# DredderGun/accbpg_and_fw

Hardware: AMD Instinct MI355X
Metric: D-opt iters/sec (m=2048,n=32768) (higher is better)
Workload: dtype f64; 1 GPU; D_opt_design(2048,32768) abpg_gain gamma=2 fp64, one independent instance per GPU; instances=1, instances_per_gpu=1, seeds=1..1, window=transient: iterations 5..161 from x0 = 1/n, linear_gram=False

## Files before the change

accbpg_and_fw_amd/_lib.py:

```python
from __future__ import annotations

import ctypes as C
import os

_HERE = os.path.dirname(os.path.abspath(__file__))
LIB_PATH = os.environ.get("ACCBPG_HIP_LIB") or os.path.join(_HERE, "lib", "libaccbpg_hip.so")

OK, ERR_ASSERT, ERR_NOT_PD, ERR_HIP, ERR_ARG = 0, 1, 2, 3, 4

_lib = None


class FwProbe(C.Structure):
    _fields_ = [("i", C.c_int64), ("j", C.c_int64), ("w_i", C.c_double), ("w_j", C.c_double),
                ("x_j", C.c_double), ("logdet_H", C.c_double), ("q_prev", C.c_double)]


class FwStep(C.Structure):
    _fields_ = [("i", C.c_int64), ("j", C.c_int64), ("w_i", C.c_double), ("w_j", C.c_double), ("x_j", C.c_double),
                ("q_prev", C.c_double), ("p", C.c_int64), ("xscale", C.c_double), ("xadd", C.c_double),
                ("hcoef", C.c_double), ("hdiv", C.c_double), ("kind", C.c_int32), ("status", C.c_int32)]


FW_RUN_MAX = 1024
# ... 94 lines not shown
    "accbpg_symnmf_func_grad": (C.c_int, [_P, _P, C.c_int, C.POINTER(C.c_double), _P]),
    "accbpg_symnmf_plan": (C.c_int, [_P, C.POINTER(C.c_int64)]),
    "accbpg_quartic_prox_stage": (C.c_int, [_P, _P, C.c_double, C.c_double, C.c_int, C.c_double, C.c_int64, _P,
                                            C.POINTER(C.c_double), _P, _P]),
    "accbpg_quartic_ls_terms": (C.c_int, [_P, _P, _P, _P, _P, C.c_int64, C.POINTER(C.c_double), _P, _P]),
    "accbpg_lmo_l2_ball": (C.c_int, [_P, C.c_int, _P, C.c_double, C.c_double, C.c_double, C.c_int64, _P,
                                     C.POINTER(C.c_double), _P, _P]),
    "accbpg_lmo_linf_ball": (C.c_int, [_P, C.c_int, _P, C.c_double, C.c_double, C.c_int64, _P, _P]),
    "accbpg_burg_reg_div_prox": (C.c_int, [C.c_int, _P, _P, C.c_double, C.c_double, C.c_int64, _P, _P]),
    "accbpg_vec_dot": (C.c_int, [_P, _P, C.c_int64, C.POINTER(C.c_double), _P, _P]),
    "accbpg_combine_ls_terms": (C.c_int, [C.c_int, C.c_double, _P, C.c_double, _P, C.c_double, _P, _P, C.c_int64, _P,
                                          C.POINTER(C.c_double), _P, _P]),
    "accbpg_burg_simplex_prox_acc": (C.c_int, [_P, C.c_double, _P, C.c_double, C.c_double, C.c_int64, _P, _P, _P,
                                               C.POINTER(C.c_int), _P]),
    "accbpg_lmo_l2_ball_pos": (C.c_int, [_P, _P, C.c_double, C.c_double, C.c_int64, _P, C.POINTER(C.c_double), _P, _P]),
    "accbpg_dopt_profile_enable": (C.c_int, [_P, C.c_int]),
    "accbpg_dopt_profile_read": (C.c_int, [_P, C.c_int, C.POINTER(C.c_double), C.POINTER(C.c_int64)]),
    "accbpg_dopt_profile_reset": (C.c_int, [_P]),
    "accbpg_debug_pipe_probe": (C.c_int, [C.c_int, C.c_int, C.POINTER(C.c_double), _P]),
    "accbpg_mfma_f64_peak": (C.c_int, [C.c_int, C.POINTER(C.c_double), _P]),
    "accbpg_dopt_factor_in_small_launches": (C.c_int, [_P, C.c_int]),
    "accbpg_debug_chol_variant": (C.c_int, [_P, C.c_int]),
    "accbpg_debug_plan_flags": (C.c_int, [C.c_int]),
    "accbpg_debug_chol_trace": (C.c_int, [_P, _P, C.c_int, C.POINTER(C.c_int64)]),
    "accbpg_debug_gram_variant": (C.c_int, [_P, _P, C.c_int, C.c_int, C.POINTER(C.c_double)]),
    "accbpg_debug_grad_variant": (C.c_int, [_P, _P, C.c_int, C.c_int, C.POINTER(C.c_double)]),
    "accbpg_test_gemm": (C.c_int, [_P, C.c_int64, _P, C.c_int64, _P, C.c_int64, C.c_int64, C.c_int64,
                                   C.c_int64, C.c_int, C.c_double, C.c_double, C.c_int, _P]),
}

EXPORTS = tuple(sorted(_SIGS))


def load():
    global _lib
    if _lib is not None:
        return _lib
    if not os.path.exists(LIB_PATH):
        raise ImportError(
            "accbpg_and_fw_amd: %s is missing -- build it with "
            "`make -C accbpg_and_fw_amd/csrc` or `python -c 'import __graft_entry__ as g; g.build()'`. "
            "There is no CPU fallback." % LIB_PATH)
    lib = C.CDLL(LIB_PATH)
    for name, (res, args) in _SIGS.items():
        fn = getattr(lib, name)
        fn.restype = res
# ... 21 lines not shown
```

accbpg_and_fw_amd/csrc/capi.hip:

```cpp
#include <stdarg.h>
#include <string.h>
#include <stdlib.h>
#include <algorithm>

#include "internal.h"
#include "reduce.hpp"

namespace accbpg {

static thread_local char g_err[512] = "";

void set_last_error(const char* fmt, ...) {
    va_list ap;
    va_start(ap, fmt);
    vsnprintf(g_err, sizeof(g_err), fmt, ap);
    va_end(ap);
}

void note_tiles_fallback(const char* where) {
    static bool said = false;
    if (said) return;
    said = true;
    fprintf(stderr, "libaccbpg_hip: %s: the one-launch Cholesky abandoned a wait (another process on this GPU, or fewer "
                    "workgroups resident than the occupancy query promised); this handle factors with one launch per block "
// ... 461 lines not shown
}

extern "C" int accbpg_test_gemm(const double* A_dev, int64_t lda, const double* B_dev, int64_t ldb, double* C_dev,
                                int64_t ldc, int64_t M, int64_t N, int64_t K, int b_kmajor, double alpha,
                                double beta, int config, void* stream) {
    if (!A_dev || !B_dev || !C_dev || M <= 0 || N <= 0 || K <= 0) return ACCBPG_ERR_ARG;
    return launch_test_gemm(A_dev, lda, B_dev, ldb, C_dev, ldc, M, N, K, b_kmajor, alpha, beta, config,
                            (hipStream_t)stream);
}

extern "C" int accbpg_dopt_factor_in_small_launches(accbpg_dopt* h, int on) {
    if (!h || on < 0 || on > 2) return ACCBPG_ERR_ARG;
    const int64_t T = (h->m + NB - 1) / NB;
    value_forget(h);
    h->chol_tiles_off = on == 1 || (on == 2 && T * (T + 1) / 2 >= h->num_cu);
    return ACCBPG_OK;
}

extern "C" int accbpg_debug_plan_flags(int flags) {
    set_plan_flags(flags);
    return ACCBPG_OK;
}

extern "C" int accbpg_debug_chol_variant(accbpg_dopt* h, int bits) {
    if (!h) return ACCBPG_ERR_ARG;
    value_forget(h);
    h->chol_dbg = bits & 63;
    h->chol_tiles_off = (bits & 64) != 0;
    if (bits & 2048) h->chol_tiles_off = true;
    h->chol_stall_test = (bits & 128) ? 1 : 0;
    h->chol_spin_limit = (bits & 128) ? 200000 : 20000000;
    h->kern_variant = (bits >> 30) & 3;
    if (bits & 256) h->use_glds = false;
    if (bits & 512) h->use_glds = true;
    if (bits & 2048) {
        h->chol_two_level_T = (bits >> 12) & 0xfff;
        if ((bits >> 24) & 0x3f) h->chol_nk = (bits >> 24) & 0x3f;
    }
    return ACCBPG_OK;
}

extern "C" int accbpg_debug_chol_trace(accbpg_dopt* h, const double* gram_dev, int with_inverse, int64_t* stamps_host) {
    if (!h || !gram_dev || !stamps_host) return ACCBPG_ERR_ARG;
    if (!chol_tiles_usable(h)) {
        set_last_error("accbpg_debug_chol_trace: the one-launch Cholesky is not in use for this handle");
        return ACCBPG_ERR_ARG;
// ... 28 lines not shown
```

accbpg_and_fw_amd/csrc/dopt_kernels.hip:

```cpp
#include <mutex>
#include <unordered_map>
#include <type_traits>

#include "internal.h"
#include "mfma_tile.hpp"

namespace accbpg {

struct GramSeg {
    int64_t row0, col0, kb, ke;
    bool dual, whole;
};
constexpr int GRAM_RMAX = 4;
template <class T>
__device__ __forceinline__ GramSeg gram_segment(const TileRC* __restrict__ tiles, int64_t kiters, int64_t it,
                                                int64_t it1) {
    const int e = (int)(it / kiters);
    const int64_t off = it - (int64_t)e * kiters;
    const TileRC tr = tiles[e];
    GramSeg g;
    if (tr.d1 < 0) {
        g.row0 = (int64_t)tr.rb * T::BM; g.col0 = (int64_t)tr.cb * T::BN;
        g.kb = off; g.ke = min(kiters, off + (it1 - it));
        g.dual = false;
// ... 757 lines not shown
template <class T, int CV = 0>
__device__ __forceinline__ void colnorm_glds_body(
    const double* __restrict__ W, int64_t ldw, const double* __restrict__ V, int64_t ldv, int64_t m, int64_t n,
    double* __restrict__ out, double sign) {
    if constexpr (CV == COLNORM_CV) colnorm_phases_body<T>(W, ldw, V, ldv, m, n, out, sign);
    else colnorm_restart_body<T, CV>(W, ldw, V, ldv, m, n, out, sign);
}

template <class T, int CV = 0>
__global__ __launch_bounds__(NTHREADS, 1) void colnorm_glds_kernel(
    const double* __restrict__ W, int64_t ldw, const double* __restrict__ V, int64_t ldv, int64_t m, int64_t n,
    double* __restrict__ out, double sign) {
    colnorm_glds_body<T, CV>(W, ldw, V, ldv, m, n, out, sign);
}
template <class T>
__global__ __launch_bounds__(NTHREADS, 1) void colnorm_glds_batch_kernel(
    const BatchInst* __restrict__ bt, BatchAct act, int64_t ldw, int64_t ldv, int64_t m, int64_t n,
    double* __restrict__ outbase, int64_t ldo, double sign) {
    const int inst = act.idx[blockIdx.y];
    const BatchInst bi = bt[inst];
    colnorm_glds_body<T, COLNORM_CV>(bi.Wbuf, ldw, bi.V, ldv, m, n, outbase + (int64_t)inst * ldo, sign);
}

template <class T>
__device__ __forceinline__ void gemm_ops_body(const GemmOp op) {
    extern __shared__ __attribute__((aligned(16))) double lds[];
    const int64_t row0 = (int64_t)blockIdx.y * T::BM, col0 = (int64_t)blockIdx.x * T::BN;
    if (row0 >= op.M || col0 >= op.N) return;
    if (op.lower_only && col0 > row0 + T::BM - 1) return;
    const bool va = ((reinterpret_cast<uintptr_t>(op.A) & 15) == 0) && ((op.lda & 1) == 0);
    const bool vb = ((reinterpret_cast<uintptr_t>(op.B) & 15) == 0) && ((op.ldb & 1) == 0);
    T t;
    t.zero();
    int64_t ksteps = (op.K + BK - 1) / BK;
    int64_t ks0 = 0;
    if (op.tri & 1) ks0 = max((int64_t)0, col0 - op.koff) / BK;
    if (op.tri & 2) ksteps = min(ksteps, max((int64_t)0, row0 + T::BM - op.koff + BK - 1) / BK);
    if (ks0 >= ksteps) {
        t.store_C(op.C, op.ldc, row0, col0, op.M, op.N, op.alpha, op.beta, op.lower_only != 0);
        return;
    }
    auto gload = [&](int64_t ks) {
        t.gload_A(op.A, op.lda, row0, op.M, ks * BK, op.K, va);
        if constexpr (T::BKM) t.gload_B_km(op.B, op.ldb, col0, op.N, ks * BK, op.K, vb);
        else t.gload_B_kc(op.B, op.ldb, col0, op.N, ks * BK, op.K, vb);
    };
    gload(ks0);
    t.sstore(lds);
    __syncthreads();
    int cur = 0;
    for (int64_t ks = ks0; ks < ksteps; ++ks) {
        const bool more = ks + 1 < ksteps;
        if (more) gload(ks + 1);
        t.compute(lds + cur * T::STAGE_ELEMS);
        if (more) t.sstore(lds + (cur ^ 1) * T::STAGE_ELEMS);
        __syncthreads();
        cur ^= 1;
    }
    t.store_C(op.C, op.ldc, row0, col0, op.M, op.N, op.alpha, op.beta, op.lower_only != 0);
}

template <class T>
__global__ __launch_bounds__(NTHREADS, 2) void gemm_ops_kernel(const GemmOp* __restrict__ ops) {
    gemm_ops_body<T>(ops[blockIdx.z]);
}
template <class T>
__global__ __launch_bounds__(NTHREADS, 2) void gemm_ops_batch_kernel(const GemmOp* __restrict__ ops, int per_inst, int begin,
                                                                    int count, BatchAct act) {
    const int a = blockIdx.z / count, o = blockIdx.z - a * count;
    gemm_ops_body<T>(ops[(int64_t)act.idx[a] * per_inst + begin + o]);
}

__device__ __forceinline__ void gemm_reduce_body(const RedOp r) {
    const int64_t total = (int64_t)r.M * r.N;
    const int64_t stride = (int64_t)gridDim.x * 256 * 2;
    for (int64_t e = 2 * ((int64_t)blockIdx.x * 256 + threadIdx.x); e < total; e += stride) {
        double2 acc = *reinterpret_cast<const double2*>(r.P + e);
        for (int p = 1; p < r.ns; ++p) {
            const double2 v = *reinterpret_cast<const double2*>(r.P + (int64_t)p * total + e);
            acc.x += v.x;
            acc.y += v.y;
        }
        const int64_t row = e / r.N, col = e - row * r.N;
        *reinterpret_cast<double2*>(r.C + row * r.ldc + col) = acc;
    }
}
__global__ __launch_bounds__(256) void gemm_reduce_kernel(const RedOp* __restrict__ reds) { gemm_reduce_body(reds[blockIdx.y]); }
__global__ __launch_bounds__(256) void gemm_reduce_batch_kernel(const RedOp* __restrict__ reds, int per_inst, int begin, int count,
                                                               BatchAct act) {
    const int a = blockIdx.y / count, o = blockIdx.y - a * count;
    gemm_reduce_body(reds[(int64_t)act.idx[a] * per_inst + begin + o]);
}

// ... 1119 lines not shown

void prof_begin(accbpg_dopt* h, ProfKind k) {
    if (!h->prof_on) return;
    ProfSlot& p = h->prof[k];
    if (p.used + 2 > p.ev.size()) {
        hipEvent_t a, b;
        hipEventCreate(&a);
        hipEventCreate(&b);
        p.ev.push_back(a);
        p.ev.push_back(b);
    }
    hipEventRecord(p.ev[p.used], h->stream);
}
void prof_end(accbpg_dopt* h, ProfKind k) {
    if (!h->prof_on) return;
    ProfSlot& p = h->prof[k];
    hipEventRecord(p.ev[p.used + 1], h->stream);
    p.used += 2;
    p.launches += 1;
}

static int g_plan_flags = 0;
void set_plan_flags(int flags) { g_plan_flags = flags; }

int build_plans(accbpg_dopt* h) {
    const int64_t m = h->m;
    const bool interior256 = h->vec_ok && (m % 256 == 0) && (h->n % BK == 0);
    const int BM = h->big ? TileBig<false>::BM : TileSmall<false>::BM;
    const int BN = h->big ? TileBig<false>::BN : TileSmall<false>::BN;
    std::vector<TileRC> tl;
    const int nrb = (int)((m + BM - 1) / BM), ncb = (int)((m + BN - 1) / BN);
    h->gram_chunks = 1;
    h->gram_nc = h->n;
    constexpr int64_t GRAM_NC = 32768;
    if (!(g_plan_flags & 4) && h->big && interior256 && h->use_glds && h->n >= 2 * GRAM_NC && h->n % GRAM_NC == 0) {
        h->gram_chunks = (int)(h->n / GRAM_NC);
        h->gram_nc = GRAM_NC;
        if (!(g_plan_flags & 8) && h->ldv * (int64_t)sizeof(double) >= (1 << 20)) {
            const size_t bytes = sizeof(double) * (size_t)m * (size_t)h->n;
            if (hipMalloc(&h->Vblk, bytes) == hipSuccess) {
                for (int c = 0; c < h->gram_chunks; ++c)
                    ACC_HIP(hipMemcpy2DAsync(h->Vblk + (size_t)c * m * GRAM_NC, sizeof(double) * GRAM_NC,
                                             h->V + (size_t)c * GRAM_NC, sizeof(double) * (size_t)h->ldv,
                                             sizeof(double) * GRAM_NC, (size_t)m, hipMemcpyDeviceToDevice, h->stream));
                ACC_HIP(hipStreamSynchronize(h->stream));
            } else {
// ... 257 lines not shown
        h->chol_tiles_grid = (int)jobs.size();
        h->chol_slots = std::min(per_cu, 2) * h->num_cu;
        h->chol_tiles_ok = per_cu >= 1 && (int64_t)jobs.size() <= (int64_t)h->chol_slots;
        if (h->chol_tiles_ok) {
            ACC_HIP(hipMalloc(&h->chol_jobs, sizeof(CholJob) * jobs.size()));
            ACC_HIP(hipMemcpy(h->chol_jobs, jobs.data(), sizeof(CholJob) * jobs.size(), hipMemcpyHostToDevice));
            ACC_HIP(hipMalloc(&h->chol_ready, sizeof(int) * (size_t)(T * T + 5 * T)));
            ACC_HIP(hipMemset(h->chol_ready, 0, sizeof(int) * (size_t)(T * T + 5 * T)));
            ACC_HIP(hipMalloc(&h->chol_hand, sizeof(double) * (size_t)T * NB * NB));
            ACC_HIP(hipMalloc(&h->chol_aux, sizeof(double) * (size_t)T * CT_AUX));
            ACC_HIP(hipMalloc(&h->Gbuf, sizeof(double) * (size_t)m * m));
            ACC_HIP(hipMemset(h->Gbuf, 0, sizeof(double) * (size_t)m * m));
        }
    }

    ACC_TRY(set_lds(gram_streamk_kernel<TileBig<false, true>>, TileBig<false>::LDS_BYTES));
    ACC_TRY(set_lds(gram_streamk_kernel<TileBig<false, false>>, TileBig<false>::LDS_BYTES));
    ACC_TRY(set_lds(gram_streamk_kernel<TileSmall<false, true>>, TileSmall<false>::LDS_BYTES));
    ACC_TRY(set_lds(gram_streamk_kernel<TileSmall<false, false>>, TileSmall<false>::LDS_BYTES));
    ACC_TRY(set_lds(colnorm_kernel<TileBig<true, true>>, TileBig<true>::LDS_BYTES));
    ACC_TRY(set_lds(colnorm_kernel<TileBig<true, false>>, TileBig<true>::LDS_BYTES));
    ACC_TRY(set_lds(colnorm_kernel<TileSmall<true, true>>, TileSmall<true>::LDS_BYTES));
    ACC_TRY(set_lds(colnorm_kernel<TileSmall<true, false>>, TileSmall<true>::LDS_BYTES));
    ACC_TRY(set_lds(gemm_ops_kernel<TileSmall<true>>, TileSmall<true>::LDS_BYTES));
    ACC_TRY(set_lds(gemm_ops_kernel<TileSmall<false>>, TileSmall<false>::LDS_BYTES));
    ACC_TRY(set_lds(chol_step_kernel, CHOL_LDS_BYTES));
    ACC_TRY(set_lds(chol_syrk_kernel, SYRK_LDS_BYTES));
    ACC_TRY(set_lds(gemm_big_kernel<TileBig<true>>, TileBig<true>::LDS_BYTES));
    ACC_TRY(set_lds(gemm_big_kernel<TileBig<false>>, TileBig<false>::LDS_BYTES));
    return ACCBPG_OK;
}

template <class T>
static int gram_launch_t(accbpg_dopt* h, const double* x, double* gram) {
    if constexpr (!T::EDGE && T::BM == 256) {
        if (h->use_glds || h->has_duals) {
            const int64_t nc = h->gram_chunks > 1 ? h->gram_nc : h->n;
            for (int c = 0; c < h->gram_chunks; ++c) {
                const double* Vc = h->Vblk ? h->Vblk + (int64_t)c * h->m * nc : h->V + (int64_t)c * nc;
                const int64_t ldc = h->Vblk ? nc : h->ldv;
                const double* xc = x + (int64_t)c * nc;
                const double beta = c == 0 ? 0.0 : 1.0;
                const int all_slabs = h->gram_chunks > 1 ? 1 : 0;
                prof_begin(h, PROF_GRAM);
#define ACC_GRAM_ARGS Vc, ldc, h->m, nc, xc, h->tiles, h->wg_ranges, h->kiters, h->gram_nslot, h->slabs, gram, h->m, all_slabs
                if (h->kern_variant == 1)
                    ACC_LAUNCH_LDS((gram_streamk_glds_kernel<T, GRAM_GV ^ 128>), h->gram_grid, NTHREADS, T::G_LDS_BYTES, h->stream, ACC_GRAM_ARGS);
                else if (h->kern_variant == 3)
// ... 104 lines not shown
        if (interior) ACC_TRY((gram_launch_t<TileSmall<false, false>>(h, x, gram)));
        else ACC_TRY((gram_launch_t<TileSmall<false, true>>(h, x, gram)));
    }
    ACC_HIP(hipGetLastError());
    return ACCBPG_OK;
}

__global__ __launch_bounds__(256) void copy_kernel(double* __restrict__ dst, const double* __restrict__ src, size_t n) {
    const size_t stride = (size_t)gridDim.x * 256;
    for (size_t i = (size_t)blockIdx.x * 256 + threadIdx.x; i < n; i += stride) dst[i] = src[i];
}
int device_copy(double* dst, const double* src, size_t ndoubles, hipStream_t s) {
    if (ndoubles == 0 || dst == src) return ACCBPG_OK;
    size_t nb = (ndoubles + 255) / 256;
    if (nb > 4096) nb = 4096;
    copy_kernel<<<(unsigned)nb, 256, 0, s>>>(dst, src, ndoubles);
    ACC_HIP(hipGetLastError());
    return ACCBPG_OK;
}

int launch_gemm_ops(const GemmOp* ops_dev, int nops, int maxM, int maxN, bool b_kmajor, hipStream_t s) {
    if (nops <= 0 || maxM <= 0 || maxN <= 0) return ACCBPG_OK;
    dim3 grid((maxN + 63) / 64, (maxM + 63) / 64, nops);
    if (b_kmajor)
        gemm_ops_kernel<TileSmall<true>><<<grid, NTHREADS, TileSmall<true>::LDS_BYTES, s>>>(ops_dev);
    else
        gemm_ops_kernel<TileSmall<false>><<<grid, NTHREADS, TileSmall<false>::LDS_BYTES, s>>>(ops_dev);
    ACC_HIP(hipGetLastError());
    return ACCBPG_OK;
}

static std::mutex g_tiles_mu;
constexpr int TILES_RING = 16;
struct TilesRing {
    hipEvent_t ev[TILES_RING] = {};
    hipStream_t stream[TILES_RING] = {};
    int grid[TILES_RING] = {};
    long long issued = 0;
};
static TilesRing g_tiles[64];

bool chol_tiles_usable(const accbpg_dopt* h) {
    return h->chol_tiles_ok && !h->chol_tiles_off && (h->chol_dbg & 63) == 0;
}

static int launch_chol_tiles(accbpg_dopt* h, const double* src, double* A, double* Winv) {
    const int64_t m = h->m;
    const int T = (int)((m + NB - 1) / NB);
    CholInst ci;
    ci.src = src; ci.L = A; ci.Ldiag = h->Tbuf; ci.Winv = Winv; ci.logdet = h->dscal; ci.flags = h->dflag;
    ci.ready = h->chol_ready; ci.aux = h->chol_aux; ci.hand = h->chol_hand; ci.trace = h->chol_trace;
    const int dev = (h->device >= 0 && h->device < 64) ? h->device : 0;
// ... 161 lines not shown
        CholInst{}, b->chol_table[with_inverse ? 1 : 0], reinterpret_cast<const CholJob*>(h0->chol_jobs), m, m, T,
        h0->chol_spin_limit, 0, act);
    prof_end(h0, PROF_CHOL);
    ACC_HIP(hipGetLastError());
    {
        const int slot = (int)(ring.issued % TILES_RING);
        if (!ring.ev[slot]) ACC_HIP(hipEventCreateWithFlags(&ring.ev[slot], hipEventDisableTiming));
        ACC_HIP(hipEventRecord(ring.ev[slot], b->stream));
        ring.stream[slot] = b->stream;
        ring.grid[slot] = grid_all;
        ++ring.issued;
    }
    return ACCBPG_OK;
}

int launch_trtri_batch(accbpg_dopt_batch* b, const BatchAct& act) {
    accbpg_dopt* h0 = b->inst[0];
    prof_begin(h0, PROF_TRTRI);
    for (const accbpg_dopt::MergeStage& st : h0->merge_stages) {
        const int count = st.end - st.begin;
        if (count <= 0) continue;
        if (st.kind == 0) {
            dim3 grid((st.maxn + 63) / 64, (st.maxm + 63) / 64, count * act.n);
            gemm_ops_batch_kernel<TileSmall<true>><<<grid, NTHREADS, TileSmall<true>::LDS_BYTES, b->stream>>>(
                b->ops_all, b->ops_per_inst, st.begin, count, act);
        } else {
            int gx = (int)std::min<int64_t>(1024, ((int64_t)st.maxm / 2 + 255) / 256);
            gemm_reduce_batch_kernel<<<dim3(gx, count * act.n), 256, 0, b->stream>>>(b->red_all, b->red_per_inst, st.begin, count, act);
        }
    }
    prof_end(h0, PROF_TRTRI);
    ACC_HIP(hipGetLastError());
    return ACCBPG_OK;
}

int debug_grad_variant(accbpg_dopt* h, double* out, int var, int iters, double* ms_out) {
    using T = TileBig<true, false>;
    const bool vw = ((reinterpret_cast<uintptr_t>(h->Wbuf) & 15) == 0) && ((h->m & 1) == 0);
    if (!h->big || !h->use_glds || !vw || !h->vec_ok || h->m % 256 != 0 || h->n % 128 != 0) return ACCBPG_ERR_ARG;
    const int grid = (int)(h->n / T::BN), lds = T::G_LDS_BYTES + 4 * T::BN * 8;
    if (var != 0 && var != 3 && (var < 10 || var > 13)) return ACCBPG_ERR_ARG;
    hipEvent_t a, b;
    ACC_HIP(hipEventCreate(&a));
    if (hipEventCreate(&b) != hipSuccess) {
        hipEventDestroy(a);
        return ACCBPG_ERR_HIP;
    }
    auto launch = [&]() -> int {
// ... 46 lines not shown
}

int launch_test_gemm(const double* A, int64_t lda, const double* B, int64_t ldb, double* C, int64_t ldc, int64_t M,
                     int64_t N, int64_t K, int b_kmajor, double alpha, double beta, int config, hipStream_t s) {
    GemmOp op{};
    op.A = A; op.B = B; op.C = C; op.lda = lda; op.ldb = ldb; op.ldc = ldc;
    op.M = (int)M; op.N = (int)N; op.K = (int)K; op.lower_only = 0; op.alpha = alpha; op.beta = beta;
    if (config == 1) {
        if (b_kmajor) {
            using T = TileBig<true>;
            ACC_TRY(set_lds(gemm_big_kernel<T>, T::LDS_BYTES));
            dim3 grid((unsigned)((N + T::BN - 1) / T::BN), (unsigned)((M + T::BM - 1) / T::BM));
            gemm_big_kernel<T><<<grid, NTHREADS, T::LDS_BYTES, s>>>(op);
        } else {
            using T = TileBig<false>;
            ACC_TRY(set_lds(gemm_big_kernel<T>, T::LDS_BYTES));
            dim3 grid((unsigned)((N + T::BN - 1) / T::BN), (unsigned)((M + T::BM - 1) / T::BM));
            gemm_big_kernel<T><<<grid, NTHREADS, T::LDS_BYTES, s>>>(op);
        }
    } else {
        GemmOp* d = nullptr;
        ACC_HIP(hipMalloc(&d, sizeof(GemmOp)));
        ACC_HIP(hipMemcpyAsync(d, &op, sizeof(GemmOp), hipMemcpyHostToDevice, s));
        ACC_TRY(set_lds(gemm_ops_kernel<TileSmall<true>>, TileSmall<true>::LDS_BYTES));
        ACC_TRY(set_lds(gemm_ops_kernel<TileSmall<false>>, TileSmall<false>::LDS_BYTES));
        int rc = launch_gemm_ops(d, 1, (int)M, (int)N, b_kmajor != 0, s);
        hipStreamSynchronize(s);
        hipFree(d);
        return rc;
    }
    ACC_HIP(hipGetLastError());
    return ACCBPG_OK;
}

int pipe_probe(int iters, int mode, double* ms_out, hipStream_t s) {
    int dev = 0;
    hipDeviceProp_t prop;
    ACC_HIP(hipGetDevice(&dev));
    ACC_HIP(hipGetDeviceProperties(&prop, dev));
    double* sink = nullptr;
    ACC_HIP(hipMalloc(&sink, 8));
    hipEvent_t a, b;
    ACC_HIP(hipEventCreate(&a));
    ACC_HIP(hipEventCreate(&b));
    pipe_probe_kernel<<<prop.multiProcessorCount, NTHREADS, 0, s>>>(iters / 10 + 1, mode, sink);
    ACC_HIP(hipEventRecord(a, s));
    pipe_probe_kernel<<<prop.multiProcessorCount, NTHREADS, 0, s>>>(iters, mode, sink);
    ACC_HIP(hipEventRecord(b, s));
// ... 36 lines not shown
```

accbpg_and_fw_amd/csrc/internal.h:

```cpp
#pragma once
#include <hip/hip_runtime.h>
#include <stdint.h>
#include <stdio.h>
#include <vector>

#include "../../include/accbpg_hip.h"

namespace accbpg {

void set_last_error(const char* fmt, ...);
void note_tiles_fallback(const char* where);

#define ACC_HIP(call)                                                                         \
    do {                                                                                      \
        hipError_t e__ = (call);                                                              \
        if (e__ != hipSuccess) {                                                              \
            ::accbpg::set_last_error("%s:%d: %s -> %s", __FILE__, __LINE__, #call,            \
                                     hipGetErrorString(e__));                                 \
            return ACCBPG_ERR_HIP;                                                            \
        }                                                                                     \
    } while (0)

#define ACC_TRY(call)                       \
    do {                                    \
// ... 260 lines not shown

namespace accbpg {

int launch_gram_batch(accbpg_dopt_batch* b, const BatchAct& act, const double* xbase, int64_t ldx);
int launch_cholesky_batch(accbpg_dopt_batch* b, const BatchAct& act, bool with_inverse, const double* xbase, int64_t ldx);
int launch_trtri_batch(accbpg_dopt_batch* b, const BatchAct& act);
int launch_colnorm_batch(accbpg_dopt_batch* b, const BatchAct& act, double* gbase, int64_t ldg, double sign);

int dopt_init(accbpg_dopt* h);
int launch_gram(accbpg_dopt* h, const double* x, double* gram);
int launch_cholesky(accbpg_dopt* h, double* A , double* Winv = nullptr ,
                    const double* xcheck = nullptr ,
                    const double* src = nullptr ,
                    double* xkeep = nullptr );
bool chol_tiles_usable(const accbpg_dopt* h);
int launch_trtri(accbpg_dopt* h);
int launch_colnorm(accbpg_dopt* h, const double* W, double* out, double sign);
int launch_gemm_ops(const GemmOp* ops_dev, int nops, int maxM, int maxN, bool b_kmajor, hipStream_t s);
int launch_test_gemm(const double* A, int64_t lda, const double* B, int64_t ldb, double* C, int64_t ldc,
                     int64_t M, int64_t N, int64_t K, int b_kmajor, double alpha, double beta, int config,
                     hipStream_t s);
int build_plans(accbpg_dopt* h);
void set_plan_flags(int flags);
int debug_gram_variant(accbpg_dopt* h, const double* x, int var, int iters, double* ms_out);
int debug_grad_variant(accbpg_dopt* h, double* out, int var, int iters, double* ms_out);
int mfma_peak(int iters, double* tflops, hipStream_t s);
int pipe_probe(int iters, int mode, double* ms_out, hipStream_t s);

int64_t vec_ws_doubles(int64_t n);
int vec_scratch(double** pin, int** flags, double** out);

int vt_nsplit(int64_t m, int64_t n, int num_cu);
int launch_vt_times(const double* V, int64_t ldv, int64_t m, int64_t n, const double* q, double* upart, int nsplit,
                    double* u, bool vec_ok, hipStream_t s);
int launch_vt_times_batch(const KyInst* tab, int K, int64_t ldv, int64_t m, int64_t n, bool first, int nsplit,
                          hipStream_t s);
constexpr int VT_MAXSPLIT = 64;

int device_copy(double* dst, const double* src, size_t ndoubles, hipStream_t s);

void prof_begin(accbpg_dopt* h, ProfKind k);
void prof_end(accbpg_dopt* h, ProfKind k);

}
```

accbpg_and_fw_amd/csrc/mfma_tile.hpp:

```cpp
#pragma once
#include <hip/hip_runtime.h>
#include <stdint.h>
#include <type_traits>

namespace accbpg {

typedef double d4 __attribute__((ext_vector_type(4)));
typedef double d2 __attribute__((ext_vector_type(2)));

constexpr int BK = 16;
constexpr int SK = BK + 2;
constexpr int NTHREADS = 256;

__device__ __forceinline__ d2 load2_guard(const double* __restrict__ p, bool row_ok, int64_t k, int64_t K,
                                          bool vec_ok) {
    d2 v;
    if (row_ok && vec_ok && k + 1 < K) {
        v = *reinterpret_cast<const d2*>(p);
    } else {
        v.x = (row_ok && k < K) ? p[0] : 0.0;
        v.y = (row_ok && k + 1 < K) ? p[1] : 0.0;
    }
    return v;
}

template <int B, int E, class F>
__device__ __forceinline__ void static_for(F&& f) {
    if constexpr (B < E) {
        f(std::integral_constant<int, B>{});
        static_for<B + 1, E>(f);
    }
}

template <int BM_, int BN_, int WM_, int WN_, bool BKM_, bool EDGE_ = true>
struct Tile {
    static constexpr bool EDGE = EDGE_;
    static constexpr int BM = BM_, BN = BN_, WM = WM_, WN = WN_;
    static constexpr bool BKM = BKM_;
    static constexpr int WAVES_M = BM / WM, WAVES_N = BN / WN;
    static_assert(WAVES_M * WAVES_N == 4, "4 waves per workgroup");
    static constexpr int MI = WM / 16, NI = WN / 16;
// ... 14 lines not shown

    __device__ __forceinline__ void zero() {
#pragma unroll
        for (int i = 0; i < MI; ++i)
#pragma unroll
            for (int j = 0; j < NI; ++j) acc[i][j] = d4{0.0, 0.0, 0.0, 0.0};
    }

    __device__ __forceinline__ void pin_acc() {
#pragma unroll
        for (int i = 0; i < MI; ++i)
#pragma unroll
            for (int j = 0; j < NI; ++j) asm volatile("" : "+a"(acc[i][j]));
    }

    __device__ __forceinline__ void pin_acc_col(int j_rt) {
#pragma unroll
        for (int i = 0; i < MI; ++i)
#pragma unroll
            for (int j = 0; j < NI; ++j)
                if (j == j_rt) asm volatile("" : "+a"(acc[i][j]));
    }

    __device__ __forceinline__ void gload_A(const double* __restrict__ A, int64_t lda, int64_t row0, int64_t M,
                                            int64_t k0, int64_t K, bool vec_ok) {
        const int tid = threadIdx.x;
        const int c = tid & 7, r = tid >> 3;
        const int64_t k = k0 + 2 * c;
        if constexpr (!EDGE) {
            const double* __restrict__ base = A + (row0 + r) * lda + k;
#pragma unroll
            for (int p = 0; p < A_PASS; ++p) ra[p] = *reinterpret_cast<const d2*>(base + (int64_t)(32 * p) * lda);
        } else {
#pragma unroll
            for (int p = 0; p < A_PASS; ++p) {
                const int64_t row = row0 + r + 32 * p;
                ra[p] = load2_guard(A + row * lda + k, row < M, k, K, vec_ok);
            }
        }
    }
    __device__ __forceinline__ void scale_A(const double* __restrict__ x, int64_t k0, int64_t K) {
        const int c = threadIdx.x & 7;
        const int64_t k = k0 + 2 * c;
        double x0, x1;
        if constexpr (!EDGE) {
            const d2 xv = *reinterpret_cast<const d2*>(x + k);
            x0 = xv.x; x1 = xv.y;
        } else {
            x0 = (k < K) ? x[k] : 0.0;
            x1 = (k + 1 < K) ? x[k + 1] : 0.0;
        }
#pragma unroll
        for (int p = 0; p < A_PASS; ++p) {
            ra[p].x *= x0;
            ra[p].y *= x1;
        }
    }
    __device__ __forceinline__ void gload_B_kc(const double* __restrict__ B, int64_t ldb, int64_t col0, int64_t N,
                                               int64_t k0, int64_t K, bool vec_ok) {
        const int tid = threadIdx.x;
        const int c = tid & 7, r = tid >> 3;
        const int64_t k = k0 + 2 * c;
        if constexpr (!EDGE) {
            const double* __restrict__ base = B + (col0 + r) * ldb + k;
#pragma unroll
            for (int p = 0; p < B_PASS; ++p) rb[p] = *reinterpret_cast<const d2*>(base + (int64_t)(32 * p) * ldb);
        } else {
#pragma unroll
            for (int p = 0; p < B_PASS; ++p) {
                const int64_t row = col0 + r + 32 * p;
                rb[p] = load2_guard(B + row * ldb + k, row < N, k, K, vec_ok);
            }
        }
    }
    __device__ __forceinline__ void gload_B_km(const double* __restrict__ B, int64_t ldb, int64_t col0, int64_t N,
                                               int64_t k0, int64_t K, bool vec_ok) {
        const int tid = threadIdx.x;
        const int c = 2 * (tid % BKM_TPR), r = tid / BKM_TPR;
        const int64_t col = col0 + c;
        if constexpr (!EDGE) {
            const double* __restrict__ base = B + (k0 + r) * ldb + col;
#pragma unroll
            for (int p = 0; p < B_PASS; ++p)
                rb[p] = *reinterpret_cast<const d2*>(base + (int64_t)(BKM_RPP * p) * ldb);
        } else {
#pragma unroll
            for (int p = 0; p < B_PASS; ++p) {
                const int64_t k = k0 + r + BKM_RPP * p;
                rb[p] = load2_guard(B + k * ldb + col, k < K, col, N, vec_ok);
            }
        }
    }

    __device__ __forceinline__ void sstore(double* __restrict__ stage) {
        const int tid = threadIdx.x;
        {
            const int c = tid & 7, r = tid >> 3;
#pragma unroll
            for (int p = 0; p < A_PASS; ++p)
                *reinterpret_cast<d2*>(stage + (r + 32 * p) * SK + 2 * c) = ra[p];
        }
        double* bs = stage + A_ELEMS;
        if constexpr (BKM) {
            const int c = 2 * (tid % BKM_TPR), r = tid / BKM_TPR;
#pragma unroll
            for (int p = 0; p < B_PASS; ++p)
                *reinterpret_cast<d2*>(bs + (r + BKM_RPP * p) * SBN + c) = rb[p];
// ... 535 lines not shown
```

include/accbpg_hip.h:

```cpp
#ifndef ACCBPG_HIP_H
#define ACCBPG_HIP_H

#include <stdint.h>

#ifdef __cplusplus
extern "C" {
#endif

#define ACCBPG_OK            0
#define ACCBPG_ERR_ASSERT    1
#define ACCBPG_ERR_NOT_PD    2
#define ACCBPG_ERR_HIP       3
#define ACCBPG_ERR_ARG       4

typedef struct accbpg_dopt accbpg_dopt;

int         accbpg_abi_version(void);
const char* accbpg_last_error(void);


int accbpg_dopt_create(const double* V_dev, int64_t m, int64_t n, int64_t ldv,
                       void* stream, accbpg_dopt** out, int is_shard);
int accbpg_dopt_destroy(accbpg_dopt* h);
int accbpg_dopt_set_stream(accbpg_dopt* h, void* stream);
// ... 218 lines not shown

int accbpg_lmo_l2_ball_pos(const double* g_dev, const double* center_dev, double radius, double epsilon, int64_t n,
                           double* out_dev, double* info3_host, double* ws_dev, void* stream);


int accbpg_dopt_profile_enable(accbpg_dopt* h, int enable);
int accbpg_dopt_profile_read(accbpg_dopt* h, int which, double* total_ms_host, int64_t* launches_host);
int accbpg_dopt_profile_reset(accbpg_dopt* h);

int accbpg_mfma_f64_peak(int iters, double* tflops_host, void* stream);

int accbpg_debug_pipe_probe(int iters, int mode, double* ms_host, void* stream);

int accbpg_test_gemm(const double* A_dev, int64_t lda, const double* B_dev, int64_t ldb,
                     double* C_dev, int64_t ldc, int64_t M, int64_t N, int64_t K,
                     int b_kmajor, double alpha, double beta, int config, void* stream);

int accbpg_debug_gram_variant(accbpg_dopt* h, const double* x_dev, int variant, int iters, double* ms_host);
int accbpg_debug_grad_variant(accbpg_dopt* h, double* g_dev, int variant, int iters, double* ms_host);
int accbpg_dopt_factor_in_small_launches(accbpg_dopt* h, int on);

int accbpg_debug_plan_flags(int flags);

int accbpg_debug_chol_variant(accbpg_dopt* h, int bits);
int accbpg_debug_chol_trace(accbpg_dopt* h, const double* gram_dev, int with_inverse, int64_t* stamps_host);

#ifdef __cplusplus
}
#endif
#endif
```

Before: 62.96 iterations/s.

## Prefetch GEMM k-steps several stages deep with register queue and unguarded interior tiles

The small-tile GEMM ops kernel now keeps a register queue of D (default 3) future k-step global loads in flight instead of a single next-step prefetch, storing from the queue into the double-buffered LDS stage. Fully interior tiles take an unguarded path with global address-space pointers and a fully unrolled steady-state group. The aim is to hide global memory latency behind MFMA compute. In exchange it adds register pressure under launch bounds of two blocks per CU, which may cause spills or lower occupancy. A debug switch selects the loop depth, including the original loop.

```diff
diff --git a/accbpg_and_fw_amd/_lib.py b/accbpg_and_fw_amd/_lib.py
--- a/accbpg_and_fw_amd/_lib.py
+++ b/accbpg_and_fw_amd/_lib.py
@@ -140,6 +140,7 @@
     "accbpg_dopt_factor_in_small_launches": (C.c_int, [_P, C.c_int]),
     "accbpg_debug_chol_variant": (C.c_int, [_P, C.c_int]),
     "accbpg_debug_plan_flags": (C.c_int, [C.c_int]),
+    "accbpg_debug_gemm_loop": (C.c_int, [C.c_int]),
     "accbpg_debug_chol_trace": (C.c_int, [_P, _P, C.c_int, C.POINTER(C.c_int64)]),
     "accbpg_debug_gram_variant": (C.c_int, [_P, _P, C.c_int, C.c_int, C.POINTER(C.c_double)]),
     "accbpg_debug_grad_variant": (C.c_int, [_P, _P, C.c_int, C.c_int, C.POINTER(C.c_double)]),
diff --git a/accbpg_and_fw_amd/csrc/capi.hip b/accbpg_and_fw_amd/csrc/capi.hip
--- a/accbpg_and_fw_amd/csrc/capi.hip
+++ b/accbpg_and_fw_amd/csrc/capi.hip
@@ -507,6 +507,10 @@
     return ACCBPG_OK;
 }
 
+extern "C" int accbpg_debug_gemm_loop(int variant) {
+    return set_gemm_loop(variant);
+}
+
 extern "C" int accbpg_debug_chol_variant(accbpg_dopt* h, int bits) {
     if (!h) return ACCBPG_ERR_ARG;
     value_forget(h);
diff --git a/accbpg_and_fw_amd/csrc/dopt_kernels.hip b/accbpg_and_fw_amd/csrc/dopt_kernels.hip
--- a/accbpg_and_fw_amd/csrc/dopt_kernels.hip
+++ b/accbpg_and_fw_amd/csrc/dopt_kernels.hip
@@ -1,3 +1,4 @@
+#include <atomic>
 #include <mutex>
 #include <unordered_map>
 #include <type_traits>
@@ -803,7 +804,7 @@
     colnorm_glds_body<T, COLNORM_CV>(bi.Wbuf, ldw, bi.V, ldv, m, n, outbase + (int64_t)inst * ldo, sign);
 }
 
-template <class T>
+template <class T, int LOOP>
 __device__ __forceinline__ void gemm_ops_body(const GemmOp op) {
     extern __shared__ __attribute__((aligned(16))) double lds[];
     const int64_t row0 = (int64_t)blockIdx.y * T::BM, col0 = (int64_t)blockIdx.x * T::BN;
@@ -821,35 +822,91 @@
         t.store_C(op.C, op.ldc, row0, col0, op.M, op.N, op.alpha, op.beta, op.lower_only != 0);
         return;
     }
-    auto gload = [&](int64_t ks) {
-        t.gload_A(op.A, op.lda, row0, op.M, ks * BK, op.K, va);
-        if constexpr (T::BKM) t.gload_B_km(op.B, op.ldb, col0, op.N, ks * BK, op.K, vb);
-        else t.gload_B_kc(op.B, op.ldb, col0, op.N, ks * BK, op.K, vb);
-    };
-    gload(ks0);
-    t.sstore(lds);
-    __syncthreads();
-    int cur = 0;
-    for (int64_t ks = ks0; ks < ksteps; ++ks) {
-        const bool more = ks + 1 < ksteps;
-        if (more) gload(ks + 1);
-        t.compute(lds + cur * T::STAGE_ELEMS);
-        if (more) t.sstore(lds + (cur ^ 1) * T::STAGE_ELEMS);
+    if constexpr (LOOP == 0) {
+        auto gload = [&](int64_t ks) {
+            t.gload_A(op.A, op.lda, row0, op.M, ks * BK, op.K, va);
+            if constexpr (T::BKM) t.gload_B_km(op.B, op.ldb, col0, op.N, ks * BK, op.K, vb);
+            else t.gload_B_kc(op.B, op.ldb, col0, op.N, ks * BK, op.K, vb);
+        };
+        gload(ks0);
+        t.sstore(lds);
         __syncthreads();
-        cur ^= 1;
+        int cur = 0;
+        for (int64_t ks = ks0; ks < ksteps; ++ks) {
+            const bool more = ks + 1 < ksteps;
+            if (more) gload(ks + 1);
+            t.compute(lds + cur * T::STAGE_ELEMS);
+            if (more) t.sstore(lds + (cur ^ 1) * T::STAGE_ELEMS);
+            __syncthreads();
+            cur ^= 1;
+        }
+    } else {
+        constexpr int D = LOOP;
+        const bool inside = va && vb && row0 + T::BM <= op.M && col0 + T::BN <= op.N && ksteps * BK <= op.K;
+        d2 pa[D][T::A_PASS], pb[D][T::B_PASS];
+        auto sstore_from = [&](auto slot, double* __restrict__ stage) {
+            constexpr int S = decltype(slot)::value;
+#pragma unroll
+            for (int p = 0; p < T::A_PASS; ++p) t.ra[p] = pa[S][p];
+#pragma unroll
+            for (int p = 0; p < T::B_PASS; ++p) t.rb[p] = pb[S][p];
+            t.sstore(stage);
+        };
+        auto run = [&](auto guard) {
+            constexpr bool GUARD = decltype(guard)::value;
+            auto gload_to = [&](auto slot, int64_t ks) {
+                constexpr int S = decltype(slot)::value;
+                t.template gload_A<GUARD>(as_global(op.A), op.lda, row0, op.M, ks * BK, op.K, va);
+                if constexpr (T::BKM) t.template gload_B_km<GUARD>(as_global(op.B), op.ldb, col0, op.N, ks * BK, op.K, vb);
+                else t.template gload_B_kc<GUARD>(as_global(op.B), op.ldb, col0, op.N, ks * BK, op.K, vb);
+#pragma unroll
+                for (int p = 0; p < T::A_PASS; ++p) pa[S][p] = t.ra[p];
+#pragma unroll
+                for (int p = 0; p < T::B_PASS; ++p) pb[S][p] = t.rb[p];
+            };
+            static_for<0, D>([&](auto j) {
+                if (ks0 + decltype(j)::value < ksteps) gload_to(j, ks0 + decltype(j)::value);
+            });
+            sstore_from(std::integral_constant<int, 0>{}, lds);
+            if (ks0 + D < ksteps) gload_to(std::integral_constant<int, 0>{}, ks0 + D);
+            __syncthreads();
+            int cur = 0;
+            auto group = [&](int64_t ks, auto full) {
+                constexpr bool FULL = decltype(full)::value;
+                static_for<0, D>([&](auto j) {
+                    constexpr int J = decltype(j)::value;
+                    const int64_t s = ks + J;
+                    if (FULL || s < ksteps) {
+                        std::integral_constant<int, (J + 1) % D> next;
+                        if (FULL || s + 1 < ksteps) sstore_from(next, lds + (cur ^ 1) * T::STAGE_ELEMS);
+                        if (FULL || s + 1 + D < ksteps) gload_to(next, s + 1 + D);
+                        t.compute(lds + cur * T::STAGE_ELEMS);
+                        __syncthreads();
+                        cur ^= 1;
+                    }
+                });
+            };
+            int64_t ks = ks0;
+            if constexpr (!GUARD)
+                for (; ks + 2 * D < ksteps; ks += D) group(ks, std::true_type{});
+            for (; ks < ksteps; ks += D) group(ks, std::false_type{});
+        };
+        if (inside) run(std::false_type{});
+        else run(std::true_type{});
     }
     t.store_C(op.C, op.ldc, row0, col0, op.M, op.N, op.alpha, op.beta, op.lower_only != 0);
 }
 
-template <class T>
+constexpr int GEMM_LOOP_DEPTH = 3;
+template <class T, int LOOP = GEMM_LOOP_DEPTH>
 __global__ __launch_bounds__(NTHREADS, 2) void gemm_ops_kernel(const GemmOp* __restrict__ ops) {
-    gemm_ops_body<T>(ops[blockIdx.z]);
-}
-template <class T>
+    gemm_ops_body<T, LOOP>(ops[blockIdx.z]);
+}
+template <class T, int LOOP = GEMM_LOOP_DEPTH>
 __global__ __launch_bounds__(NTHREADS, 2) void gemm_ops_batch_kernel(const GemmOp* __restrict__ ops, int per_inst, int begin,
                                                                     int count, BatchAct act) {
     const int a = blockIdx.z / count, o = blockIdx.z - a * count;
-    gemm_ops_body<T>(ops[(int64_t)act.idx[a] * per_inst + begin + o]);
+    gemm_ops_body<T, LOOP>(ops[(int64_t)act.idx[a] * per_inst + begin + o]);
 }
 
 __device__ __forceinline__ void gemm_reduce_body(const RedOp r) {
@@ -2015,6 +2072,36 @@
 
 static int g_plan_flags = 0;
 void set_plan_flags(int flags) { g_plan_flags = flags; }
+
+static std::atomic<int> g_gemm_loop{0};
+int set_gemm_loop(int variant) {
+    if (variant < 0 || variant > 4) return ACCBPG_ERR_ARG;
+    g_gemm_loop.store(variant);
+    return ACCBPG_OK;
+}
+template <int LOOP>
+static int set_lds_gemm_loop() {
+    ACC_TRY(set_lds(gemm_ops_kernel<TileSmall<true>, LOOP>, TileSmall<true>::LDS_BYTES));
+    ACC_TRY(set_lds(gemm_ops_kernel<TileSmall<false>, LOOP>, TileSmall<false>::LDS_BYTES));
+    return ACCBPG_OK;
+}
+static int set_lds_gemm_ops() {
+    ACC_TRY(set_lds_gemm_loop<0>());
+    ACC_TRY(set_lds_gemm_loop<2>());
+    ACC_TRY(set_lds_gemm_loop<3>());
+    ACC_TRY(set_lds_gemm_loop<4>());
+    return ACCBPG_OK;
+}
+template <class F>
+static int with_gemm_loop(F&& f) {
+    switch (g_gemm_loop.load()) {
+        case 0: return f(std::integral_constant<int, GEMM_LOOP_DEPTH>{});
+        case 1: return f(std::integral_constant<int, 0>{});
+        case 2: return f(std::integral_constant<int, 2>{});
+        case 3: return f(std::integral_constant<int, 3>{});
+        default: return f(std::integral_constant<int, 4>{});
+    }
+}
 
 int build_plans(accbpg_dopt* h) {
     const int64_t m = h->m;
@@ -2318,8 +2405,7 @@
     ACC_TRY(set_lds(colnorm_kernel<TileBig<true, false>>, TileBig<true>::LDS_BYTES));
     ACC_TRY(set_lds(colnorm_kernel<TileSmall<true, true>>, TileSmall<true>::LDS_BYTES));
     ACC_TRY(set_lds(colnorm_kernel<TileSmall<true, false>>, TileSmall<true>::LDS_BYTES));
-    ACC_TRY(set_lds(gemm_ops_kernel<TileSmall<true>>, TileSmall<true>::LDS_BYTES));
-    ACC_TRY(set_lds(gemm_ops_kernel<TileSmall<false>>, TileSmall<false>::LDS_BYTES));
+    ACC_TRY(set_lds_gemm_ops());
     ACC_TRY(set_lds(chol_step_kernel, CHOL_LDS_BYTES));
     ACC_TRY(set_lds(chol_syrk_kernel, SYRK_LDS_BYTES));
     ACC_TRY(set_lds(gemm_big_kernel<TileBig<true>>, TileBig<true>::LDS_BYTES));
@@ -2470,12 +2556,15 @@
 int launch_gemm_ops(const GemmOp* ops_dev, int nops, int maxM, int maxN, bool b_kmajor, hipStream_t s) {
     if (nops <= 0 || maxM <= 0 || maxN <= 0) return ACCBPG_OK;
     dim3 grid((maxN + 63) / 64, (maxM + 63) / 64, nops);
-    if (b_kmajor)
-        gemm_ops_kernel<TileSmall<true>><<<grid, NTHREADS, TileSmall<true>::LDS_BYTES, s>>>(ops_dev);
-    else
-        gemm_ops_kernel<TileSmall<false>><<<grid, NTHREADS, TileSmall<false>::LDS_BYTES, s>>>(ops_dev);
-    ACC_HIP(hipGetLastError());
-    return ACCBPG_OK;
+    return with_gemm_loop([&](auto loop) -> int {
+        constexpr int LOOP = decltype(loop)::value;
+        if (b_kmajor)
+            gemm_ops_kernel<TileSmall<true>, LOOP><<<grid, NTHREADS, TileSmall<true>::LDS_BYTES, s>>>(ops_dev);
+        else
+            gemm_ops_kernel<TileSmall<false>, LOOP><<<grid, NTHREADS, TileSmall<false>::LDS_BYTES, s>>>(ops_dev);
+        ACC_HIP(hipGetLastError());
+        return ACCBPG_OK;
+    });
 }
 
 static std::mutex g_tiles_mu;
@@ -2683,8 +2772,11 @@
         if (count <= 0) continue;
         if (st.kind == 0) {
             dim3 grid((st.maxn + 63) / 64, (st.maxm + 63) / 64, count * act.n);
-            gemm_ops_batch_kernel<TileSmall<true>><<<grid, NTHREADS, TileSmall<true>::LDS_BYTES, b->stream>>>(
-                b->ops_all, b->ops_per_inst, st.begin, count, act);
+            ACC_TRY(with_gemm_loop([&](auto loop) -> int {
+                gemm_ops_batch_kernel<TileSmall<true>, decltype(loop)::value><<<grid, NTHREADS, TileSmall<true>::LDS_BYTES, b->stream>>>(
+                    b->ops_all, b->ops_per_inst, st.begin, count, act);
+                return ACCBPG_OK;
+            }));
         } else {
             int gx = (int)std::min<int64_t>(1024, ((int64_t)st.maxm / 2 + 255) / 256);
             gemm_reduce_batch_kernel<<<dim3(gx, count * act.n), 256, 0, b->stream>>>(b->red_all, b->red_per_inst, st.begin, count, act);
@@ -2777,8 +2869,7 @@
         GemmOp* d = nullptr;
         ACC_HIP(hipMalloc(&d, sizeof(GemmOp)));
         ACC_HIP(hipMemcpyAsync(d, &op, sizeof(GemmOp), hipMemcpyHostToDevice, s));
-        ACC_TRY(set_lds(gemm_ops_kernel<TileSmall<true>>, TileSmall<true>::LDS_BYTES));
-        ACC_TRY(set_lds(gemm_ops_kernel<TileSmall<false>>, TileSmall<false>::LDS_BYTES));
+        ACC_TRY(set_lds_gemm_ops());
         int rc = launch_gemm_ops(d, 1, (int)M, (int)N, b_kmajor != 0, s);
         hipStreamSynchronize(s);
         hipFree(d);
diff --git a/accbpg_and_fw_amd/csrc/internal.h b/accbpg_and_fw_amd/csrc/internal.h
--- a/accbpg_and_fw_amd/csrc/internal.h
+++ b/accbpg_and_fw_amd/csrc/internal.h
@@ -306,6 +306,7 @@
                      hipStream_t s);
 int build_plans(accbpg_dopt* h);
 void set_plan_flags(int flags);
+int set_gemm_loop(int variant);
 int debug_gram_variant(accbpg_dopt* h, const double* x, int var, int iters, double* ms_out);
 int debug_grad_variant(accbpg_dopt* h, double* out, int var, int iters, double* ms_out);
 int mfma_peak(int iters, double* tflops, hipStream_t s);
diff --git a/accbpg_and_fw_amd/csrc/mfma_tile.hpp b/accbpg_and_fw_amd/csrc/mfma_tile.hpp
--- a/accbpg_and_fw_amd/csrc/mfma_tile.hpp
+++ b/accbpg_and_fw_amd/csrc/mfma_tile.hpp
@@ -12,11 +12,16 @@
 constexpr int SK = BK + 2;
 constexpr int NTHREADS = 256;
 
-__device__ __forceinline__ d2 load2_guard(const double* __restrict__ p, bool row_ok, int64_t k, int64_t K,
-                                          bool vec_ok) {
+typedef const __attribute__((address_space(1))) double* gptr;
+__device__ __forceinline__ gptr as_global(const double* p) { return (gptr)p; }
+__device__ __forceinline__ d2 ld2(const double* p) { return *reinterpret_cast<const d2*>(p); }
+__device__ __forceinline__ d2 ld2(gptr p) { return *(const __attribute__((address_space(1))) d2*)p; }
+
+template <class P>
+__device__ __forceinline__ d2 load2_guard(P p, bool row_ok, int64_t k, int64_t K, bool vec_ok) {
     d2 v;
     if (row_ok && vec_ok && k + 1 < K) {
-        v = *reinterpret_cast<const d2*>(p);
+        v = ld2(p);
     } else {
         v.x = (row_ok && k < K) ? p[0] : 0.0;
         v.y = (row_ok && k + 1 < K) ? p[1] : 0.0;
@@ -77,15 +82,16 @@
                 if (j == j_rt) asm volatile("" : "+a"(acc[i][j]));
     }
 
-    __device__ __forceinline__ void gload_A(const double* __restrict__ A, int64_t lda, int64_t row0, int64_t M,
+    template <bool GUARD = EDGE_, class P>
+    __device__ __forceinline__ void gload_A(P __restrict__ A, int64_t lda, int64_t row0, int64_t M,
                                             int64_t k0, int64_t K, bool vec_ok) {
         const int tid = threadIdx.x;
         const int c = tid & 7, r = tid >> 3;
         const int64_t k = k0 + 2 * c;
-        if constexpr (!EDGE) {
-            const double* __restrict__ base = A + (row0 + r) * lda + k;
-#pragma unroll
-            for (int p = 0; p < A_PASS; ++p) ra[p] = *reinterpret_cast<const d2*>(base + (int64_t)(32 * p) * lda);
+        if constexpr (!GUARD) {
+            P __restrict__ base = A + (row0 + r) * lda + k;
+#pragma unroll
+            for (int p = 0; p < A_PASS; ++p) ra[p] = ld2(base + (int64_t)(32 * p) * lda);
         } else {
 #pragma unroll
             for (int p = 0; p < A_PASS; ++p) {
@@ -111,15 +117,16 @@
             ra[p].y *= x1;
         }
     }
-    __device__ __forceinline__ void gload_B_kc(const double* __restrict__ B, int64_t ldb, int64_t col0, int64_t N,
+    template <bool GUARD = EDGE_, class P>
+    __device__ __forceinline__ void gload_B_kc(P __restrict__ B, int64_t ldb, int64_t col0, int64_t N,
                                                int64_t k0, int64_t K, bool vec_ok) {
         const int tid = threadIdx.x;
         const int c = tid & 7, r = tid >> 3;
         const int64_t k = k0 + 2 * c;
-        if constexpr (!EDGE) {
-            const double* __restrict__ base = B + (col0 + r) * ldb + k;
-#pragma unroll
-            for (int p = 0; p < B_PASS; ++p) rb[p] = *reinterpret_cast<const d2*>(base + (int64_t)(32 * p) * ldb);
+        if constexpr (!GUARD) {
+            P __restrict__ base = B + (col0 + r) * ldb + k;
+#pragma unroll
+            for (int p = 0; p < B_PASS; ++p) rb[p] = ld2(base + (int64_t)(32 * p) * ldb);
         } else {
 #pragma unroll
             for (int p = 0; p < B_PASS; ++p) {
@@ -128,16 +135,17 @@
             }
         }
     }
-    __device__ __forceinline__ void gload_B_km(const double* __restrict__ B, int64_t ldb, int64_t col0, int64_t N,
+    template <bool GUARD = EDGE_, class P>
+    __device__ __forceinline__ void gload_B_km(P __restrict__ B, int64_t ldb, int64_t col0, int64_t N,
                                                int64_t k0, int64_t K, bool vec_ok) {
         const int tid = threadIdx.x;
         const int c = 2 * (tid % BKM_TPR), r = tid / BKM_TPR;
         const int64_t col = col0 + c;
-        if constexpr (!EDGE) {
-            const double* __restrict__ base = B + (k0 + r) * ldb + col;
+        if constexpr (!GUARD) {
+            P __restrict__ base = B + (k0 + r) * ldb + col;
 #pragma unroll
             for (int p = 0; p < B_PASS; ++p)
-                rb[p] = *reinterpret_cast<const d2*>(base + (int64_t)(BKM_RPP * p) * ldb);
+                rb[p] = ld2(base + (int64_t)(BKM_RPP * p) * ldb);
         } else {
 #pragma unroll
             for (int p = 0; p < B_PASS; ++p) {
diff --git a/include/accbpg_hip.h b/include/accbpg_hip.h
--- a/include/accbpg_hip.h
+++ b/include/accbpg_hip.h
@@ -264,6 +264,8 @@
 
 int accbpg_debug_plan_flags(int flags);
 
+int accbpg_debug_gemm_loop(int variant);
+
 int accbpg_debug_chol_variant(accbpg_dopt* h, int bits);
 int accbpg_debug_chol_trace(accbpg_dopt* h, const double* gram_dev, int with_inverse, int64_t* stamps_host);
 
```

Result: faster. 63.67 iterations/s, median of 6 (+1.1%).
